# autosome-ru/pasio

Hardware: NVIDIA B200
Metric: whole-contig segmentation throughput, default pasio pipeline (nt/s); DP cell updates/s in dp_cells_per_s (higher is better)
Workload: dtype f64

## Files before the change

include/pasio_b200.h:

```cpp
#ifndef PASIO_B200_H
#define PASIO_B200_H

#include <stdint.h>

#ifdef __cplusplus
extern "C" {
#endif

typedef struct pasio_ctx pasio_ctx;

typedef enum pasio_status {
    PASIO_OK = 0,
    PASIO_E_CUDA = -1,
    PASIO_E_ARG = -2,
    PASIO_E_COUNTS = -3,
    PASIO_E_CANDIDATES = -4,
    PASIO_E_TABLE_TOO_SHORT = -5,
    PASIO_E_STATE = -6,
    PASIO_E_TOO_LARGE = -7,
    PASIO_E_NOMEM = -8
} pasio_status;

enum { PASIO_TAB_LOG = 0,
       PASIO_TAB_LGAMMA = 1,
       PASIO_TAB_LGAMMA_ALPHA = 2   };

enum { PASIO_CONSTRAINT_NONE = 0, PASIO_CONSTRAINT_ZEROS = 1, PASIO_CONSTRAINT_CONSTANTS = 2 };

enum { PASIO_TUNE_WINDOW_PRUNE = 0,
       PASIO_TUNE_WINDOW_PHASES = 1,
       PASIO_TUNE_EXACT_PRUNE = 2,
       PASIO_TUNE_EXACT_LAG = 3,
       PASIO_TUNE_EXACT_RING = 4,
       PASIO_TUNE_LOGFAC_EXACT = 5,
       PASIO_TUNE_WINDOW_SPECULATE = 6,
       PASIO_TUNE_UPLOAD_NARROW = 7,
       PASIO_TUNE_LOGFAC_EAGER = 8,
       PASIO_TUNE_EXACT_NBLOCK = 9,
       PASIO_TUNE_COUNT = 10 };

int pasio_ctx_create(int device, pasio_ctx **out);
int pasio_ctx_destroy(pasio_ctx *ctx);
const char *pasio_last_error(const pasio_ctx *ctx);
int pasio_abi_version(void);

int pasio_set_params(pasio_ctx *ctx, int alpha_is_int, double alpha, double beta,
                     double segment_creation_cost);
int pasio_table_upload(pasio_ctx *ctx, int table_id, const double *values, int64_t n);
int pasio_table_need(const pasio_ctx *ctx, int64_t *n_log, int64_t *n_lgamma, int64_t *n_lgamma_alpha);

int pasio_contig_load(pasio_ctx *ctx, const int64_t *counts, int64_t n,
                      const int64_t *offsets, int64_t n_contigs);
int pasio_contig_load_rle(pasio_ctx *ctx, const int64_t *starts, const int64_t *values,
                          int64_t n_runs, const int64_t *offsets, int64_t n_contigs);
// ... 2 lines not shown

int pasio_contig_load_device(pasio_ctx *ctx, const int64_t *d_counts_device, int64_t n,
                             const int64_t *offsets, int64_t n_contigs);
int pasio_contig_info(const pasio_ctx *ctx, int64_t *n, int64_t *total_count, int64_t *n_contigs);
int pasio_cumsum_at(pasio_ctx *ctx, const int64_t *positions, int64_t m, int64_t *out);

int pasio_candidates_set(pasio_ctx *ctx, const int64_t *cands, int64_t m);
int pasio_candidates_count(const pasio_ctx *ctx, int64_t *m);
int pasio_candidates_download(pasio_ctx *ctx, int64_t *out, int64_t capacity, int64_t *m);

int pasio_filter_candidates(pasio_ctx *ctx, int constraint, int64_t *n_in, int64_t *n_out);

int pasio_round(pasio_ctx *ctx, int64_t window_size, int64_t window_shift, int constraint,
                int64_t *n_in, int64_t *n_out, int64_t *cells);
int pasio_round_stats(const pasio_ctx *ctx, int64_t *cells, int64_t *cells_skipped);
int pasio_exact_task_plan(int64_t n_candidates, int lag, int nblock, int32_t *triples, int64_t cap, int64_t *n_tasks);
int pasio_upload_stats(const pasio_ctx *ctx, int64_t *wire_bytes);
int pasio_set_tuning(pasio_ctx *ctx, int key, int value);
int pasio_rounds(pasio_ctx *ctx, int64_t window_size, int64_t window_shift, int constraint,
                 int64_t max_rounds, int64_t *rounds_done, int64_t *n_out, int64_t *cells,
                 int64_t *sizes, int64_t sizes_cap);
int pasio_set_penalties(pasio_ctx *ctx, const double *split_number_penalty, int64_t n_split_number_penalty,
                        double first_column_refund, const double *length_penalty, int64_t n_length_penalty);

int pasio_square_split(pasio_ctx *ctx, int64_t *out_splits, int64_t cap, int64_t *n_splits,
                       double *score, double *prefix_scores, int64_t *previous_splits);
int pasio_square_split_regularized(pasio_ctx *ctx, const double *length_penalty, int64_t n_length_penalty,
                                   const double *split_number_penalty, int64_t n_split_number_penalty,
                                   double first_column_refund, int64_t *out_splits, int64_t cap, int64_t *n_splits,
                                   double *score, double *prefix_scores, int64_t *previous_splits);
// ... 40 lines not shown
```

pasio_b200/_native.py:

```python
import ctypes
import os
import threading

import numpy as np

_HERE = os.path.dirname(os.path.abspath(__file__))
LIB_PATH = os.environ.get('PASIO_B200_LIB') or os.path.join(_HERE, 'libpasio_b200.so')

OK = 0
E_CUDA, E_ARG, E_COUNTS, E_CANDIDATES, E_TABLE_TOO_SHORT, E_STATE, E_TOO_LARGE, E_NOMEM = range(-1, -9, -1)
TAB_LOG, TAB_LGAMMA, TAB_LGAMMA_ALPHA = 0, 1, 2
CONSTRAINTS = {'none': 0, 'zeros': 1, 'constants': 2}
TUNE = {'window_prune': 0, 'window_phases': 1, 'exact_prune': 2, 'exact_lag': 3, 'exact_ring': 4, 'logfac_exact': 5,
        'window_speculate': 6, 'upload_narrow': 7,
        'logfac_eager': 8, 'exact_nblock': 9}
TIMING_FAMILIES = ['scan', 'window_dp', 'compact', 'exact_dp', 'score', 'h2d', 'd2h']

_i64 = ctypes.c_int64
_i64p = ctypes.POINTER(ctypes.c_int64)
_f64p = ctypes.POINTER(ctypes.c_double)
_vp = ctypes.c_void_p

SIGNATURES = {
    'pasio_ctx_create': (ctypes.c_int, [ctypes.c_int, ctypes.POINTER(_vp)]),
    'pasio_ctx_destroy': (ctypes.c_int, [_vp]),
    'pasio_last_error': (ctypes.c_char_p, [_vp]),
    'pasio_abi_version': (ctypes.c_int, []),
    'pasio_set_params': (ctypes.c_int, [_vp, ctypes.c_int, ctypes.c_double, ctypes.c_double, ctypes.c_double]),
    'pasio_table_upload': (ctypes.c_int, [_vp, ctypes.c_int, _f64p, _i64]),
    'pasio_table_need': (ctypes.c_int, [_vp, _i64p, _i64p, _i64p]),
    'pasio_contig_load': (ctypes.c_int, [_vp, _i64p, _i64, _i64p, _i64]),
    'pasio_contig_load_round': (ctypes.c_int, [_vp, _i64p, _i64, _i64, _i64, ctypes.c_int, _i64p, _i64p, _i64p]),
    'pasio_contig_load_rle': (ctypes.c_int, [_vp, _i64p, _i64p, _i64, _i64p, _i64]),
    'pasio_contig_load_device': (ctypes.c_int, [_vp, _vp, _i64, _i64p, _i64]),
    'pasio_contig_info': (ctypes.c_int, [_vp, _i64p, _i64p, _i64p]),
    'pasio_cumsum_at': (ctypes.c_int, [_vp, _i64p, _i64, _i64p]),
    'pasio_candidates_set': (ctypes.c_int, [_vp, _i64p, _i64]),
    'pasio_candidates_count': (ctypes.c_int, [_vp, _i64p]),
    'pasio_candidates_download': (ctypes.c_int, [_vp, _i64p, _i64, _i64p]),
    'pasio_filter_candidates': (ctypes.c_int, [_vp, ctypes.c_int, _i64p, _i64p]),
    'pasio_round': (ctypes.c_int, [_vp, _i64, _i64, ctypes.c_int, _i64p, _i64p, _i64p]),
    'pasio_round_stats': (ctypes.c_int, [_vp, _i64p, _i64p]),
    'pasio_exact_task_plan': (ctypes.c_int, [_i64, ctypes.c_int, ctypes.c_int, ctypes.POINTER(ctypes.c_int32), _i64, _i64p]),
    'pasio_upload_stats': (ctypes.c_int, [_vp, _i64p]),
    'pasio_set_tuning': (ctypes.c_int, [_vp, ctypes.c_int, ctypes.c_int]),
    'pasio_rounds': (ctypes.c_int, [_vp, _i64, _i64, ctypes.c_int, _i64, _i64p, _i64p, _i64p, _i64p, _i64]),
    'pasio_set_penalties': (ctypes.c_int, [_vp, _f64p, _i64, ctypes.c_double, _f64p, _i64]),
    'pasio_square_split': (ctypes.c_int, [_vp, _i64p, _i64, _i64p, _f64p, _f64p, _i64p]),
    'pasio_square_split_regularized': (ctypes.c_int, [_vp, _f64p, _i64, _f64p, _i64, ctypes.c_double, _i64p, _i64, _i64p, _f64p,
                                                     _f64p, _i64p]),
    'pasio_suffix_scores': (ctypes.c_int, [_vp, _i64, _f64p]),
    'pasio_segment_scores': (ctypes.c_int, [_vp, _f64p, _i64p, _f64p, _f64p, _i64, _i64p]),
    'pasio_segment_scores_sum': (ctypes.c_int, [_vp, _f64p]),
    'pasio_segment_lmm': (ctypes.c_int, [_vp, _f64p, _i64, _f64p]),
    'pasio_logfac_prefetch': (ctypes.c_int, [_vp]),
    'pasio_host_alloc': (ctypes.c_int, [_i64, ctypes.POINTER(_vp)]),
    'pasio_host_free': (ctypes.c_int, [_vp]),
# ... 323 lines not shown
        return n_in.value, n_out.value, cells.value

    def set_tuning(self, key, value):
        self._check(self.lib.pasio_set_tuning(self.ctx, TUNE[key], int(value)))

    def upload_stats(self):
        b = _i64(0)
        self._check(self.lib.pasio_upload_stats(self.ctx, ctypes.byref(b)))
        return b.value

    def round_stats(self):
        a, b = _i64(0), _i64(0)
        self._check(self.lib.pasio_round_stats(self.ctx, ctypes.byref(a), ctypes.byref(b)))
        return a.value, b.value

    def rounds(self, window_size, window_shift, constraint, num_rounds=None, first=None):
        n, _, _ = self.info()
        limit = max(1, n if num_rounds is None else num_rounds)
        self._cands_obj = None
        sizes, cells_total = [], 0
        if first is not None:
            sizes.append(first[0])
            cells_total += first[2]
            limit -= 1
            if first[0] == first[1] or limit == 0:
                return sizes, self.candidate_count(), cells_total
        while limit > 0:
            done, n_out, cells = _i64(0), _i64(0), _i64(0)
            buf = np.zeros(64, dtype=np.int64)
            step = min(limit, 64)
# ... 232 lines not shown
```

pasio_b200/csrc/api.cu:

```cuda
#include "common.cuh"

#include <algorithm>
#include <thread>
#include <atomic>
#include <chrono>
#include <memory>
#include <cstdarg>
#include <cstdlib>
#include <cstdio>
#include <cstring>

static thread_local std::string g_create_error;

int pasio_fail(pasio_ctx *ctx, int code, const char *fmt, ...)
{
    char buf[512];
    va_list ap;
    va_start(ap, fmt);
    vsnprintf(buf, sizeof buf, fmt, ap);
    va_end(ap);
    if (ctx) ctx->err = buf; else g_create_error = buf;
    return code;
}

// ... 372 lines not shown
    if (e != cudaSuccess) return pasio_fail(nullptr, PASIO_E_CUDA, "cudaSetDevice: %s", cudaGetErrorString(e));
    pasio_ctx *ctx = new pasio_ctx();
    ctx->device = device;
    ctx->sm_count = prop.multiProcessorCount;
    ctx->smem_optin = (int)prop.sharedMemPerBlockOptin;
    int prio_lo = 0, prio_hi = 0;
    cudaDeviceGetStreamPriorityRange(&prio_lo, &prio_hi);
    if (cudaStreamCreateWithPriority(&ctx->stream, cudaStreamNonBlocking, prio_hi) != cudaSuccess ||
        cudaStreamCreateWithPriority(&ctx->stream2, cudaStreamNonBlocking, 0) != cudaSuccess ||
        cudaStreamCreateWithFlags(&ctx->stream_copy, cudaStreamNonBlocking) != cudaSuccess ||
        cudaStreamCreateWithPriority(&ctx->stream_lx, cudaStreamNonBlocking, 0) != cudaSuccess ||
        cudaEventCreateWithFlags(&ctx->ev_lx0, cudaEventDisableTiming) != cudaSuccess ||
        cudaEventCreateWithFlags(&ctx->ev_lx1, cudaEventDisableTiming) != cudaSuccess ||
        cudaEventCreateWithFlags(&ctx->ev_fork, cudaEventDisableTiming) != cudaSuccess ||
        cudaEventCreateWithFlags(&ctx->ev_join, cudaEventDisableTiming) != cudaSuccess ||
        cudaMallocHost((void **)&ctx->h_scalars, 16 * sizeof(i64)) != cudaSuccess ||
        pasio_reserve(ctx, ctx->scalars, 16 * sizeof(i64)) != PASIO_OK) {
        g_create_error = "context allocation failed: " + ctx->err;
        delete ctx;
        return PASIO_E_CUDA;
    }
    memset(ctx->h_scalars, 0, 16 * sizeof(i64));
    auto env_int = [](const char *name, int dflt) { const char *v = getenv(name); return v ? atoi(v) : dflt; };
    ctx->tune[PASIO_TUNE_WINDOW_PRUNE] = env_int("PASIO_WD_PRUNE", 1);
    ctx->tune[PASIO_TUNE_WINDOW_PHASES] = env_int("PASIO_WD_PHASES", 1);
    ctx->tune[PASIO_TUNE_EXACT_PRUNE] = env_int("PASIO_XD_PRUNE", 1);
    ctx->tune[PASIO_TUNE_EXACT_LAG] = env_int("PASIO_XD_LAG", 5);
    ctx->tune[PASIO_TUNE_EXACT_RING] = env_int("PASIO_XD_RING", 1);
    ctx->tune[PASIO_TUNE_LOGFAC_EXACT] = env_int("PASIO_B200_EXACT_LMM", 1);
    ctx->tune[PASIO_TUNE_WINDOW_SPECULATE] = env_int("PASIO_WD_SPECULATE", 1);
    ctx->tune[PASIO_TUNE_UPLOAD_NARROW] = env_int("PASIO_B200_UPLOAD_NARROW", 1);
    ctx->tune[PASIO_TUNE_LOGFAC_EAGER] = env_int("PASIO_B200_LOGFAC_EAGER", 0);
    ctx->tune[PASIO_TUNE_EXACT_NBLOCK] = env_int("PASIO_XD_NBLOCK", 3);
    if (ctx->tune[PASIO_TUNE_EXACT_LAG] < 3 || ctx->tune[PASIO_TUNE_EXACT_LAG] > 5) ctx->tune[PASIO_TUNE_EXACT_LAG] = 5;
    *out = ctx;
    return PASIO_OK;
}

extern "C" int pasio_ctx_destroy(pasio_ctx *ctx)
{
    if (!ctx) return PASIO_OK;
    cudaSetDevice(ctx->device);
    cudaStreamSynchronize(ctx->stream);
    drop_borrowed_counts(ctx);
    DevBuf *bufs[] = {&ctx->tab[0], &ctx->tab[1], &ctx->tab[2], &ctx->counts, &ctx->cg, &ctx->cpbits, &ctx->keepbits,
                      &ctx->bounds, &ctx->brank, &ctx->cand[0], &ctx->cand[1], &ctx->candC[0], &ctx->candC[1], &ctx->win_st, &ctx->win_en, &ctx->win_small, &ctx->win_medium, &ctx->win_large, &ctx->win_flags,
                      &ctx->blocksum, &ctx->tilestate, &ctx->scalars, &ctx->dpL, &ctx->dpC, &ctx->dpP, &ctx->dpPrev,
                      &ctx->dpPart, &ctx->dpPartArg, &ctx->dpMark, &ctx->dpJump, &ctx->fscan, &ctx->logfac_full,
// ... 123 lines not shown
    ctx->n_contigs = n_contigs;
    const size_t bit_bytes = (size_t)((n + 1 + 4095) / 4096) * 512 + 16;
    PASIO_TRY(pasio_reserve(ctx, ctx->cg, (size_t)(n + 2) * 8));
    PASIO_TRY(pasio_reserve(ctx, ctx->cpbits, bit_bytes));
    PASIO_TRY(pasio_reserve(ctx, ctx->keepbits, bit_bytes));
    PASIO_TRY(pasio_reserve(ctx, ctx->bounds, (size_t)(n_contigs + 1) * 4));
    PASIO_TRY(pasio_reserve(ctx, ctx->brank, (size_t)(n_contigs + 1) * 4));
    PASIO_TRY(h2d(ctx, ctx->bounds.p, ctx->h_bounds.data(), (size_t)(n_contigs + 1) * 4));
    PASIO_TRY(launch_scan_counts(ctx));
    PASIO_TRY(d2h(ctx, ctx->h_scalars, ctx->scalars.p, 3 * sizeof(i64)));
    if (ctx->h_scalars[1]) return pasio_fail(ctx, PASIO_E_COUNTS, "counts must be >= 0");
    ctx->total = ctx->h_scalars[0];
    ctx->max_count = ctx->h_scalars[2];
    ctx->have_contig = true;
    ctx->implicit_all = true;
    ctx->m = n + 1;
    ctx->cur = 0;
    PASIO_TRY(launch_boundary_ranks(ctx));
    ctx->h_brank = ctx->h_bounds;
    return PASIO_OK;
}

static int check_load_args(pasio_ctx *ctx, int64_t n, const int64_t *offsets, int64_t n_contigs)
{
    if (ctx->logfac_pending) {
        cudaStreamSynchronize(ctx->stream_lx);
        ctx->logfac_pending = false;
    }
    ctx->logfac_ready = false;
    ctx->logfac_eager = false;
// ... 100 lines not shown
    PASIO_TRY(pasio_reserve(ctx, ctx->counts, (size_t)n * 8 + 16));
    ctx->h_bounds.assign({0, (int32_t)n});
    ctx->n_contigs = 1;
    const size_t bit_alloc = (size_t)((n + 1 + 4095) / 4096) * 512 + 16;
    PASIO_TRY(pasio_reserve(ctx, ctx->cg, (size_t)(n + 2) * 8));
    PASIO_TRY(pasio_reserve(ctx, ctx->cpbits, bit_alloc));
    PASIO_TRY(pasio_reserve(ctx, ctx->keepbits, bit_alloc));
    PASIO_TRY(pasio_reserve(ctx, ctx->bounds, 2 * 4));
    PASIO_TRY(pasio_reserve(ctx, ctx->brank, 2 * 4));
    PASIO_TRY(h2d(ctx, ctx->bounds.p, ctx->h_bounds.data(), 2 * 4));
    const size_t bit_bytes = (size_t)((n + 1 + 31) / 32 + 2) * 4;
    CUDA_TRY(ctx, cudaMemsetAsync(ctx->keepbits.p, 0, bit_bytes, ctx->stream));
    i64 n_tiles = 0, tile_elems = 0;
    PASIO_TRY(launch_scan_prepare(ctx, &n_tiles, &tile_elems));
    ctx->implicit_all = true;
    ctx->m = n + 1;
    ctx->cur = 0;
    ctx->n_small = ctx->n_medium = ctx->n_large = -1;

    const i64 chunk_tiles = (i64)(32 << 20) / tile_elems;
    const i64 n_chunks = (n_tiles + chunk_tiles - 1) / chunk_tiles;
    while ((i64)ctx->chunk_events.size() < n_chunks) {
        cudaEvent_t e;
        CUDA_TRY(ctx, cudaEventCreateWithFlags(&e, cudaEventDisableTiming));
        ctx->chunk_events.push_back(e);
    }
    CUDA_TRY(ctx, cudaEventRecord(ctx->ev_fork, ctx->stream));
    CUDA_TRY(ctx, cudaStreamWaitEvent(ctx->stream_copy, ctx->ev_fork, 0));
    i64 queued = 0;
    auto queue_copies = [&](i64 upto) -> int {
// ... 103 lines not shown
        ctx->logfac_pending = true;
        ctx->logfac_eager = true;
    }
    PASIO_TRY(launch_boundary_ranks(ctx));
    ctx->h_brank = ctx->h_bounds;
    if (n_in) *n_in = ctx->m;
    if (n_out) *n_out = ctx->m;
    if (cells) *cells = 0;
    if (table_rc != PASIO_OK) return table_rc;

    const int nxt = 1 - ctx->cur;
    PASIO_TRY(pasio_reserve(ctx, ctx->cand[nxt], (size_t)ctx->m * 4));
    i64 m_new = 0;
    PASIO_TRY(launch_compact_keepbits(ctx, nxt, &m_new));
    PASIO_TRY(d2h(ctx, ctx->h_scalars + 10, ctx->scalars.as<i64>() + 10, 24));
    if (cells) *cells = ctx->h_scalars[10];
    ctx->last_cells = ctx->h_scalars[10];
    ctx->last_cells_skipped = ctx->h_scalars[12];
    ctx->cur = nxt;
    ctx->implicit_all = false;
    ctx->m = m_new;
    if (n_out) *n_out = m_new;
    return refresh_boundary_ranks(ctx);
}

extern "C" int pasio_contig_info(const pasio_ctx *ctx, int64_t *n, int64_t *total_count, int64_t *n_contigs)
{
    if (!ctx || !ctx->have_contig) return PASIO_E_STATE;
    if (n) *n = ctx->n;
    if (total_count) *total_count = ctx->total;
    if (n_contigs) *n_contigs = ctx->n_contigs;
    return PASIO_OK;
}
// ... 29 lines not shown

static int refresh_boundary_ranks(pasio_ctx *ctx)
{
    PASIO_TRY(launch_boundary_ranks(ctx));
    if (ctx->n_contigs > 1) {
        ctx->h_brank.resize((size_t)ctx->n_contigs + 1);
        PASIO_TRY(d2h(ctx, ctx->h_brank.data(), ctx->brank.p, (size_t)(ctx->n_contigs + 1) * 4));
    }
    return PASIO_OK;
}

extern "C" int pasio_candidates_set(pasio_ctx *ctx, const int64_t *cands, int64_t m)
{
    NEED_CTX(ctx);
    if (!ctx->have_contig) return pasio_fail(ctx, PASIO_E_STATE, "no contig loaded");
    if (!cands) {
        ctx->implicit_all = true;
        ctx->m = ctx->n + 1;
        return refresh_boundary_ranks(ctx);
    }
    if (m < 2 || m > ctx->n + 1) return pasio_fail(ctx, PASIO_E_CANDIDATES, "need 2 <= len(candidates) <= n+1");
    PASIO_TRY(pasio_reserve(ctx, ctx->dpJump, (size_t)m * 8));
    PASIO_TRY(pasio_reserve(ctx, ctx->cand[ctx->cur], (size_t)m * 4));
    PASIO_TRY(h2d(ctx, ctx->dpJump.p, cands, (size_t)m * 8));
    i64 *d_bad = ctx->scalars.as<i64>() + 5;
    CUDA_TRY(ctx, cudaMemsetAsync(d_bad, 0, 8, ctx->stream));
    narrow_candidates_kernel<<<ctx->sm_count * 4, 256, 0, ctx->stream>>>(ctx->dpJump.as<i64>(), m, ctx->n,
                                                                        ctx->cand[ctx->cur].as<int32_t>(), d_bad);
    CUDA_TRY(ctx, cudaGetLastError());
    PASIO_TRY(d2h(ctx, ctx->h_scalars + 5, d_bad, 8));
    if (ctx->h_scalars[5]) { ctx->implicit_all = true; ctx->m = ctx->n + 1; return pasio_fail(ctx, PASIO_E_CANDIDATES, "candidate out of range"); }
    ctx->implicit_all = false;
    ctx->m = m;
    PASIO_TRY(pasio_reserve(ctx, ctx->candC[ctx->cur], (size_t)m * 8));
    PASIO_TRY(launch_gather_i64(ctx, ctx->cg.as<i64>(), ctx->cand[ctx->cur].as<int32_t>(), nullptr, m, ctx->candC[ctx->cur].as<i64>()));
    PASIO_TRY(refresh_boundary_ranks(ctx));
    i64 bad = 0;
    PASIO_TRY(launch_validate_candidates(ctx, &bad));
    if (bad) {
        ctx->implicit_all = true;
        ctx->m = ctx->n + 1;
        refresh_boundary_ranks(ctx);
        return pasio_fail(ctx, PASIO_E_CANDIDATES,
                          "candidates must start at 0, end at len(counts), ascend strictly and contain every contig boundary");
    }
    return PASIO_OK;
}

extern "C" int pasio_candidates_count(const pasio_ctx *ctx, int64_t *m)
{
    if (!ctx || !ctx->have_contig || !m) return PASIO_E_STATE;
    *m = ctx->m;
    return PASIO_OK;
}

// ... 12 lines not shown
    if (capacity < ctx->m) return pasio_fail(ctx, PASIO_E_ARG, "capacity %lld < %lld candidates", (long long)capacity, (long long)ctx->m);
    PASIO_TRY(pasio_reserve(ctx, ctx->dpJump, (size_t)ctx->m * 8));
    widen_candidates_kernel<<<ctx->sm_count * 4, 256, 0, ctx->stream>>>(cur_cand(ctx), ctx->m, ctx->dpJump.as<i64>());
    CUDA_TRY(ctx, cudaGetLastError());
    return d2h(ctx, out, ctx->dpJump.p, (size_t)ctx->m * 8);
}

extern "C" int pasio_filter_candidates(pasio_ctx *ctx, int constraint, int64_t *n_in, int64_t *n_out)
{
    NEED_CTX(ctx);
    if (!ctx->have_contig) return pasio_fail(ctx, PASIO_E_STATE, "no contig loaded");
    if (ctx->n_contigs != 1) return pasio_fail(ctx, PASIO_E_STATE, "pasio_filter_candidates works on a single-contig context");
    if (constraint < 0 || constraint > 2) return pasio_fail(ctx, PASIO_E_ARG, "unknown constraint %d", constraint);
    if (n_in) *n_in = ctx->m;
    PASIO_TRY(launch_filter_candidates(ctx, constraint));
    const int nxt = 1 - ctx->cur;
    PASIO_TRY(pasio_reserve(ctx, ctx->cand[nxt], (size_t)ctx->m * 4));
    i64 m_new = 0;
    PASIO_TRY(launch_compact_keepbits(ctx, nxt, &m_new));
    ctx->cur = nxt;
    ctx->implicit_all = false;
    ctx->m = m_new;
    if (n_out) *n_out = m_new;
    return refresh_boundary_ranks(ctx);
}

static int build_window_table(pasio_ctx *ctx, i64 wsize, i64 wshift, i64 *nwin_out)
{
    if (ctx->n_contigs == 1) {
        *nwin_out = (ctx->m - 1 + wshift - 1) / wshift;
// ... 47 lines not shown
                          "contig total %lld / length %lld (m=%lld, implicit=%d, windows=%lld)", (long long)max_cnt,
                          (long long)max_span, (long long)ctx->total, (long long)ctx->n, (long long)ctx->m,
                          (int)ctx->implicit_all, (long long)nwin);
    PASIO_TRY(check_dp_tables(ctx, max_span, max_cnt, true));

    const size_t bit_bytes = (size_t)((ctx->n + 1 + 31) / 32 + 2) * 4;
    CUDA_TRY(ctx, cudaMemsetAsync(ctx->keepbits.p, 0, bit_bytes, ctx->stream));
    if (penalties_on(ctx)) PASIO_TRY(launch_window_dp_reg(ctx, nwin, (int)window_size, (int)window_shift, constraint));
    else PASIO_TRY(launch_window_dp(ctx, nwin, (int)window_size, (int)window_shift, constraint));

    const int nxt = 1 - ctx->cur;
    PASIO_TRY(pasio_reserve(ctx, ctx->cand[nxt], (size_t)ctx->m * 4));
    i64 m_new = 0;
    PASIO_TRY(launch_compact_keepbits(ctx, nxt, &m_new));
    PASIO_TRY(d2h(ctx, ctx->h_scalars + 10, ctx->scalars.as<i64>() + 10, 24));
    if (cells) *cells = ctx->h_scalars[10];
    ctx->last_cells = ctx->h_scalars[10];
    ctx->last_cells_skipped = ctx->h_scalars[12];
    ctx->cur = nxt;
    ctx->implicit_all = false;
    ctx->m = m_new;
    if (n_out) *n_out = m_new;
    return refresh_boundary_ranks(ctx);
}

extern "C" int pasio_rounds(pasio_ctx *ctx, int64_t window_size, int64_t window_shift, int constraint,
                            int64_t max_rounds, int64_t *rounds_done, int64_t *n_out, int64_t *cells,
                            int64_t *sizes, int64_t sizes_cap)
{
    NEED_CTX(ctx);
    if (!ctx->have_contig) return pasio_fail(ctx, PASIO_E_STATE, "no contig loaded");
    i64 limit = max_rounds <= 0 ? ctx->n : max_rounds;
    if (limit < 1) limit = 1;
// ... 17 lines not shown
extern "C" int pasio_upload_stats(const pasio_ctx *ctx, int64_t *wire_bytes)
{
    if (!ctx || !wire_bytes) return PASIO_E_ARG;
    *wire_bytes = ctx->last_wire_bytes;
    return PASIO_OK;
}

extern "C" int pasio_round_stats(const pasio_ctx *ctx, int64_t *cells, int64_t *cells_skipped)
{
    if (!ctx) return PASIO_E_ARG;
    if (cells) *cells = ctx->last_cells;
    if (cells_skipped) *cells_skipped = ctx->last_cells_skipped;
    return PASIO_OK;
}

extern "C" int pasio_set_tuning(pasio_ctx *ctx, int key, int value)
{
    if (!ctx) return PASIO_E_ARG;
    if (key < 0 || key >= PASIO_TUNE_COUNT) return pasio_fail(ctx, PASIO_E_ARG, "unknown tuning key %d", key);
    if (key == PASIO_TUNE_EXACT_LAG && (value < 3 || value > 5)) return pasio_fail(ctx, PASIO_E_ARG, "exact lag must be 3, 4 or 5");
    ctx->tune[key] = value;
    if (key == PASIO_TUNE_LOGFAC_EXACT) {
        if (ctx->logfac_pending) { cudaStreamSynchronize(ctx->stream_lx); ctx->logfac_pending = false; }
        ctx->logfac_ready = false;
        ctx->logfac_eager = false;
    }
    return PASIO_OK;
}

static int finish_square_split(pasio_ctx *ctx, i64 N, int64_t *out_splits, int64_t cap, int64_t *n_splits, double *score,
                               double *prefix_scores, int64_t *previous_splits)
{
    if (score) PASIO_TRY(d2h(ctx, score, ctx->dpP.as<double>() + (N - 1), 8));
    if (prefix_scores) PASIO_TRY(d2h(ctx, prefix_scores, ctx->dpP.p, (size_t)N * 8));
    if (previous_splits) {
        std::vector<int> tmp((size_t)N);
        PASIO_TRY(d2h(ctx, tmp.data(), ctx->dpPrev.p, (size_t)N * 4));
        for (i64 k = 0; k < N; ++k) previous_splits[k] = tmp[(size_t)k];
    }
    PASIO_TRY(launch_backtrace_mark(ctx, N));
    const int nxt = 1 - ctx->cur;
    PASIO_TRY(pasio_reserve(ctx, ctx->cand[nxt], (size_t)N * 4));
    i64 m_new = 0;
    PASIO_TRY(launch_compact_keepbits(ctx, nxt, &m_new));
    ctx->cur = nxt;
    ctx->implicit_all = false;
    ctx->m = m_new;
    PASIO_TRY(refresh_boundary_ranks(ctx));
    if (n_splits) *n_splits = m_new;
    if (out_splits) {
        if (cap < m_new) return pasio_fail(ctx, PASIO_E_ARG, "capacity %lld < %lld splits", (long long)cap, (long long)m_new);
        return pasio_candidates_download(ctx, out_splits, cap, nullptr);
    }
    return PASIO_OK;
}
// ... 314 lines not shown
```

pasio_b200/csrc/common.cuh:

```cuda
#pragma once

#include <cuda_runtime.h>
#include <stdint.h>
#include <string>
#include <vector>

#include "../../include/pasio_b200.h"

typedef long long i64;
typedef unsigned long long u64;

#define PASIO_ABI_VERSION 1

struct DevBuf {
    void *p = nullptr;
    size_t bytes = 0;
    template <typename T> T *as() const { return reinterpret_cast<T *>(p); }
};

enum TimingFamily { TF_SCAN = 0, TF_WINDOW_DP = 1, TF_COMPACT = 2, TF_EXACT_DP = 3, TF_SCORE = 4,
                    TF_H2D = 5, TF_D2H = 6, TF_COUNT = 7 };

struct TimedSpan { int family; cudaEvent_t a, b; };

// ... 62 lines not shown
    DevBuf blocksum, tilestate, scalars, dpL, dpC, dpP, dpPrev, dpPart, dpPartArg, dpMark, dpJump, fscan, logfac_full;
    DevBuf xpRing, xpRec, xpTasks, regLR, regNR;

    bool pen_num = false, pen_len = false;
    DevBuf penNR, penLR;
    i64 n_pen_nr = 0, n_pen_lr = 0;
    double pen_refund = 0.0;
    DevBuf lxPos, lxSum, lxFirst, lxState;
    i64 lx_terms = 0;
    i64 scan_tiles_done = 0;

    int tune[PASIO_TUNE_COUNT];
    i64 *h_scalars = nullptr;

    i64 last_cells = 0, last_cells_skipped = 0;
    std::vector<i64> pw_leaf_start;
    i64 pw_n = -1;
    std::vector<double> pw_leaf_sum;

    bool timing = false;
    std::vector<TimedSpan> spans;
    std::vector<cudaEvent_t> event_pool;
    double fam_ms[TF_COUNT] = {0};
    i64 fam_launches[TF_COUNT] = {0};
};

int pasio_fail(pasio_ctx *ctx, int code, const char *fmt, ...);
int pasio_reserve(pasio_ctx *ctx, DevBuf &b, size_t bytes);

#define CUDA_TRY(ctx, call)                                                                     \
// ... 99 lines not shown
```

pasio_b200/csrc/window_dp.cu:

```cuda
#include "dp_core.cuh"
#include "bound.cuh"
#include <cstdio>
#include <cstdlib>

namespace {

constexpr int WD_THREADS = 256;
constexpr int WD_WARPS = WD_THREADS / 32;
constexpr int WD_FARW = WD_WARPS - 1;
constexpr int NEAR_Q = 4;
constexpr int PR_CB = 32;
constexpr int PR_FB = 8;
constexpr int PR_MIN_N = 256;
constexpr int PR_DENSE = 28;

#ifdef PASIO_WD_PROF
__device__ unsigned long long g_wd_prof[16];
struct ProfAcc { long long t0; long long a0, a1, a2, a3, a4, a5, a6, a7; };
#define PROF_DECL ProfAcc prof = {clock64(), 0, 0, 0, 0, 0, 0, 0, 0}
__device__ __forceinline__ long long prof_clock()
{
    unsigned dummy;
    long long t;
    asm volatile("ld.volatile.shared.u32 %0, [%1];" : "=r"(dummy) : "r"(0u) : "memory");
// ... 30 lines not shown
    int constraint;
    int alpha_int;
    double alpha;
    double pen;
    int cap;
    u64 *cells;
    u64 *cells_skipped;
    unsigned *work_counter;
    const int32_t *list;
    i64 w_begin;
    i64 n_p1, list_len;
    unsigned char *done_flags;
    int p1_stride;
    int skip_covered;
    int speculate;
    int n_lg;
};

__host__ __device__ inline size_t window_smem_bytes(int cap)
{
    const size_t capr = (size_t)((cap + 31) & ~31);
    return capr * 16
           + NEAR_Q * 32 * 8
           + DP_JB * DP_JB * 8
           + NEAR_Q * 32 * 4
           + 24 * 4
           + capr * 2
           + (capr / PR_CB) * sizeof(CoarseRec)
           + 2 * 32 * sizeof(float4)
           + capr * 2
// ... 265 lines not shown
            }
        }
    }
#pragma unroll
    for (int kk = 0; kk < NK; ++kk) {
        const int k = w7 + kk * NW;
        if (k < lane && jb + lane < N) sTri[k * DP_JB + lane] = w[kk];
    }
}

__device__ __forceinline__ void build_coarse_record(int jb, const ColRec *sCol, CoarseRec *rec, double tilt_scale_c,
                                                    double tilt_scale_l)
{
    const ColRec me = sCol[jb + (threadIdx.x & 31)];
    fit_column_record(me.C, me.L, me.P, rec, tilt_scale_c, tilt_scale_l);
}

template <bool AI, int U, int RPL, bool PRUNE>
__global__ void __launch_bounds__(WD_THREADS, 3)
window_dp_kernel(WinDpParams p)
{
    extern __shared__ __align__(16) unsigned char smem[];
    const int capr = (p.cap + 31) & ~31;
    ColRec *sCol = reinterpret_cast<ColRec *>(smem);
    double *sPartV = reinterpret_cast<double *>(sCol + capr);
    double *sTri = sPartV + NEAR_Q * 32;
    int *sPartA = reinterpret_cast<int *>(sTri + DP_JB * DP_JB);
    int *sMisc = sPartA + NEAR_Q * 32;
    unsigned short *sPrev = reinterpret_cast<unsigned short *>(sMisc + 24);
    CoarseRec *sCoarse = reinterpret_cast<CoarseRec *>(sPrev + capr);
// ... 157 lines not shown
            const int par = ((jbn - 1) / DP_JB) & 1;
            const double delta_path = (sScal[0] + sScal[1] + fabs(p.pen) * DP_JB) * 1.8189894035458565e-12;
            compute_row_lb<AI>(jbn - DP_JB, jbn, N, sCol, sRow + 32 * par, sScal + 4 + par, delta_path, p.pen, p.gtab, p.ltab,
                               p.alpha_int, p.alpha);
            if (lane == 0) { sListCount[4 * par] = 0; sListCount[4 * par + 1] = 0; sListCount[4 * par + 2] = 0; }
        };
        auto run_far = [&](int jbf) {
            const int kf = (jbf - 1) / DP_JB, par = kf & 1;
            skipped += far_pass<AI>(jbf, N, kf - 1, sCol, sCoarse, sRow + 32 * par, sScal[4 + par], sList, sList + capr,
                                    sList + capr + capr / PR_CB + 8, sListCount + 4 * par, sFarV + (par * WD_FARW + warp - 1) * 32,
                                    sFarA + (par * WD_FARW + warp - 1) * 32,
                                    far_delta(), p.gtab, p.ltab, p.alpha_int, p.alpha PROF_PASS);
        };
        int jb = 1;
        const bool pipelined = PRUNE && N > PR_MIN_N && p.cand != nullptr;
        for (; jb < N && (!pipelined || jb < 1 + 2 * DP_JB); jb += DP_JB) {
            dp_block_step<AI, WD_WARPS, U, RPL>(jb, N, 0, sCol, sPrev, nullptr, sPartV, sPartA, sTri,
                                                p.gtab, p.ltab, p.alpha_int, p.alpha, p.pen, -INFINITY, 0, 0);
            if (pipelined && warp == 0) finish_block(jb);
        }
        PROF_T(6);
        if (pipelined && jb < N) {
            int spec_wait = 0, spec_back = 1;
            if (warp == 0) prepare_rows(jb);
            __syncthreads();
            if (warp > 0) run_far(jb);
            else if (jb + DP_JB < N) prepare_rows(jb + DP_JB);
            __syncthreads();
            for (; jb < N; jb += DP_JB) {
                const int k = (jb - 1) / DP_JB, buf = k & 1;
// ... 21 lines not shown
                        --spec_wait;
                    }
                    if (!resolved) block_chain<NEAR_Q>(jb, N, sCol, sPrev, nullptr, sPartV, sPartA, sTri, p.pen, ib, ia, 0, nullptr);
                    __syncwarp();
                    finish_block(jb);
                    if (jb + 2 * DP_JB < N) prepare_rows(jb + 2 * DP_JB);
                } else if (jb + DP_JB < N) {
                    run_far(jb + DP_JB);
                }
                PROF_T(2);
                __syncthreads();
                PROF_T(7);
            }
        }

        for (int k = tid; k < N; k += WD_THREADS) sMark[k] = (k == N - 1);
        __syncthreads();
        unsigned short *ja = sPrev, *jb2 = sJump;
        for (int reach = 1; reach < N; reach <<= 1) {
            for (int k = tid; k < N; k += WD_THREADS)
                if (sMark[k]) sMark[ja[k]] = 1;
            for (int k = tid; k < N; k += WD_THREADS) jb2[k] = ja[ja[k]];
            __syncthreads();
            unsigned short *t = ja; ja = jb2; jb2 = t;
        }
        int every = N == nq;
        for (int k = tid; k < N; k += WD_THREADS) {
            if (sMark[k]) {
                const i64 pos = first + sCol[k].L;
                atomicOr(p.keepbits + (pos >> 5), 1u << (pos & 31));
            } else {
                every = 0;
            }
        }
// ... 197 lines not shown
    p.ltab = ctx->tab[PASIO_TAB_LOG].as<double>();
    p.constraint = constraint;
    p.alpha_int = (int)ctx->alpha_int;
    p.alpha = ctx->alpha;
    p.pen = ctx->pen;
    i64 cap = (i64)wsize + 1;
    if (cap > ctx->m) cap = ctx->m;
    if (cap > 8192 || window_smem_bytes((int)cap) > (size_t)ctx->smem_optin)
        return pasio_fail(ctx, PASIO_E_TOO_LARGE, "window of %lld candidates does not fit one CTA's shared memory (max %d)",
                          (long long)cap, window_dp_max_candidates(ctx));
    p.cap = (int)cap;
    p.cells = ctx->scalars.as<u64>() + 10;
    p.cells_skipped = ctx->scalars.as<u64>() + 12;
    p.work_counter = ctx->scalars.as<unsigned>() + 2 * 11;
    p.w_begin = w_begin;
    if (keep_cell_counters) CUDA_TRY(ctx, cudaMemsetAsync(ctx->scalars.as<u64>() + 11, 0, 8, ctx->stream));
    else CUDA_TRY(ctx, cudaMemsetAsync(ctx->scalars.as<u64>() + 10, 0, 24, ctx->stream));
    CUDA_TRY(ctx, cudaMemsetAsync(ctx->scalars.as<u64>() + 15, 0, 8, ctx->stream));

    static const int small_env = getenv("PASIO_WD_SMALL") ? atoi(getenv("PASIO_WD_SMALL")) : 1;
    const int phase_env = ctx->tune[PASIO_TUNE_WINDOW_PHASES];
    const bool use_lists = small_env && ctx->n_small + ctx->n_medium + ctx->n_large == nwin;
    const i64 n_small = use_lists ? ctx->n_small : 0, n_medium = use_lists ? ctx->n_medium : 0;
    const i64 n_large = use_lists ? ctx->n_large : nwin;
    p.list = use_lists ? ctx->win_large.as<int32_t>() : nullptr;
    p.nwin = n_large;
    p.list_len = nwin;
    p.n_p1 = use_lists ? ctx->n_large_p1 : n_large;
    p.skip_covered = phase_env;
    p.speculate = ctx->tune[PASIO_TUNE_WINDOW_SPECULATE];
    p.done_flags = ctx->win_flags.as<unsigned char>();
    p.p1_stride = wshift > 0 && wsize / wshift > 1 ? wsize / wshift : 1;
    if (!use_lists) p.skip_covered = 0;
    ctx->n_small = ctx->n_medium = ctx->n_large = ctx->n_large_p1 = -1;
    TimingScope ts_all(ctx, TF_WINDOW_DP, 0);
    const bool fork = n_small + n_medium > 0 && n_small + n_medium <= 64;
    const bool serial_small = n_small + n_medium > 64;
    if (fork) CUDA_TRY(ctx, cudaEventRecord(ctx->ev_fork, ctx->stream));

    auto launch_small = [&](auto kern, const int32_t *list, i64 n, int nwarps, int ctas, size_t smem_bytes, unsigned *counter,
                            cudaStream_t stream) -> int {
        if (n <= 0) return PASIO_OK;
        WinDpParams ps = p;
        ps.list = list;
        ps.nwin = n;
// ... 84 lines not shown
```

Baseline: 5.706 billion.

## Certify windows where every candidate stays a split, skipping full DP

Adds a certification pass to the pruned window DP. It tries to prove that, in a near-converged round, each candidate's best predecessor is the one right before it. It checks this with coarse and fine bounds plus exact checks on the rows that survive pruning. If the window passes, the full DP and backtrace pointer-jumping are skipped and all candidates are kept. If it fails, the DP resumes from the block where it failed. The pass is enabled by default only when the previous round removed less than 1% of candidates, and it adds per-window overhead plus extra certify-stat counters and a d2h copy.

```diff
diff --git a/include/pasio_b200.h b/include/pasio_b200.h
--- a/include/pasio_b200.h
+++ b/include/pasio_b200.h
@@ -37,7 +37,8 @@
        PASIO_TUNE_UPLOAD_NARROW = 7,
        PASIO_TUNE_LOGFAC_EAGER = 8,
        PASIO_TUNE_EXACT_NBLOCK = 9,
-       PASIO_TUNE_COUNT = 10 };
+       PASIO_TUNE_WINDOW_CERTIFY = 10,
+       PASIO_TUNE_COUNT = 11 };
 
 int pasio_ctx_create(int device, pasio_ctx **out);
 int pasio_ctx_destroy(pasio_ctx *ctx);
@@ -70,6 +71,7 @@
 int pasio_round(pasio_ctx *ctx, int64_t window_size, int64_t window_shift, int constraint,
                 int64_t *n_in, int64_t *n_out, int64_t *cells);
 int pasio_round_stats(const pasio_ctx *ctx, int64_t *cells, int64_t *cells_skipped);
+int pasio_round_certify_stats(const pasio_ctx *ctx, int64_t *passed, int64_t *fell_back, int64_t *resume_rows_sum);
 int pasio_exact_task_plan(int64_t n_candidates, int lag, int nblock, int32_t *triples, int64_t cap, int64_t *n_tasks);
 int pasio_upload_stats(const pasio_ctx *ctx, int64_t *wire_bytes);
 int pasio_set_tuning(pasio_ctx *ctx, int key, int value);
diff --git a/pasio_b200/_native.py b/pasio_b200/_native.py
--- a/pasio_b200/_native.py
+++ b/pasio_b200/_native.py
@@ -13,7 +13,7 @@
 CONSTRAINTS = {'none': 0, 'zeros': 1, 'constants': 2}
 TUNE = {'window_prune': 0, 'window_phases': 1, 'exact_prune': 2, 'exact_lag': 3, 'exact_ring': 4, 'logfac_exact': 5,
         'window_speculate': 6, 'upload_narrow': 7,
-        'logfac_eager': 8, 'exact_nblock': 9}
+        'logfac_eager': 8, 'exact_nblock': 9, 'window_certify': 10}
 TIMING_FAMILIES = ['scan', 'window_dp', 'compact', 'exact_dp', 'score', 'h2d', 'd2h']
 
 _i64 = ctypes.c_int64
@@ -41,6 +41,7 @@
     'pasio_filter_candidates': (ctypes.c_int, [_vp, ctypes.c_int, _i64p, _i64p]),
     'pasio_round': (ctypes.c_int, [_vp, _i64, _i64, ctypes.c_int, _i64p, _i64p, _i64p]),
     'pasio_round_stats': (ctypes.c_int, [_vp, _i64p, _i64p]),
+    'pasio_round_certify_stats': (ctypes.c_int, [_vp, _i64p, _i64p, _i64p]),
     'pasio_exact_task_plan': (ctypes.c_int, [_i64, ctypes.c_int, ctypes.c_int, ctypes.POINTER(ctypes.c_int32), _i64, _i64p]),
     'pasio_upload_stats': (ctypes.c_int, [_vp, _i64p]),
     'pasio_set_tuning': (ctypes.c_int, [_vp, ctypes.c_int, ctypes.c_int]),
@@ -394,6 +395,11 @@
         self._check(self.lib.pasio_round_stats(self.ctx, ctypes.byref(a), ctypes.byref(b)))
         return a.value, b.value
 
+    def round_certify_stats(self):
+        a, b, c = _i64(0), _i64(0), _i64(0)
+        self._check(self.lib.pasio_round_certify_stats(self.ctx, ctypes.byref(a), ctypes.byref(b), ctypes.byref(c)))
+        return a.value, b.value, c.value
+
     def rounds(self, window_size, window_shift, constraint, num_rounds=None, first=None):
         n, _, _ = self.info()
         limit = max(1, n if num_rounds is None else num_rounds)
diff --git a/pasio_b200/csrc/api.cu b/pasio_b200/csrc/api.cu
--- a/pasio_b200/csrc/api.cu
+++ b/pasio_b200/csrc/api.cu
@@ -410,13 +410,13 @@
         cudaEventCreateWithFlags(&ctx->ev_lx1, cudaEventDisableTiming) != cudaSuccess ||
         cudaEventCreateWithFlags(&ctx->ev_fork, cudaEventDisableTiming) != cudaSuccess ||
         cudaEventCreateWithFlags(&ctx->ev_join, cudaEventDisableTiming) != cudaSuccess ||
-        cudaMallocHost((void **)&ctx->h_scalars, 16 * sizeof(i64)) != cudaSuccess ||
-        pasio_reserve(ctx, ctx->scalars, 16 * sizeof(i64)) != PASIO_OK) {
+        cudaMallocHost((void **)&ctx->h_scalars, 20 * sizeof(i64)) != cudaSuccess ||
+        pasio_reserve(ctx, ctx->scalars, 20 * sizeof(i64)) != PASIO_OK) {
         g_create_error = "context allocation failed: " + ctx->err;
         delete ctx;
         return PASIO_E_CUDA;
     }
-    memset(ctx->h_scalars, 0, 16 * sizeof(i64));
+    memset(ctx->h_scalars, 0, 20 * sizeof(i64));
     auto env_int = [](const char *name, int dflt) { const char *v = getenv(name); return v ? atoi(v) : dflt; };
     ctx->tune[PASIO_TUNE_WINDOW_PRUNE] = env_int("PASIO_WD_PRUNE", 1);
     ctx->tune[PASIO_TUNE_WINDOW_PHASES] = env_int("PASIO_WD_PHASES", 1);
@@ -428,6 +428,7 @@
     ctx->tune[PASIO_TUNE_UPLOAD_NARROW] = env_int("PASIO_B200_UPLOAD_NARROW", 1);
     ctx->tune[PASIO_TUNE_LOGFAC_EAGER] = env_int("PASIO_B200_LOGFAC_EAGER", 0);
     ctx->tune[PASIO_TUNE_EXACT_NBLOCK] = env_int("PASIO_XD_NBLOCK", 3);
+    ctx->tune[PASIO_TUNE_WINDOW_CERTIFY] = env_int("PASIO_WD_CERTIFY", 1);
     if (ctx->tune[PASIO_TUNE_EXACT_LAG] < 3 || ctx->tune[PASIO_TUNE_EXACT_LAG] > 5) ctx->tune[PASIO_TUNE_EXACT_LAG] = 5;
     *out = ctx;
     return PASIO_OK;
@@ -581,6 +582,7 @@
     ctx->max_count = ctx->h_scalars[2];
     ctx->have_contig = true;
     ctx->implicit_all = true;
+    ctx->prev_round_in = 0;
     ctx->m = n + 1;
     ctx->cur = 0;
     PASIO_TRY(launch_boundary_ranks(ctx));
@@ -711,6 +713,7 @@
     i64 n_tiles = 0, tile_elems = 0;
     PASIO_TRY(launch_scan_prepare(ctx, &n_tiles, &tile_elems));
     ctx->implicit_all = true;
+    ctx->prev_round_in = 0;
     ctx->m = n + 1;
     ctx->cur = 0;
     ctx->n_small = ctx->n_medium = ctx->n_large = -1;
@@ -844,9 +847,13 @@
     i64 m_new = 0;
     PASIO_TRY(launch_compact_keepbits(ctx, nxt, &m_new));
     PASIO_TRY(d2h(ctx, ctx->h_scalars + 10, ctx->scalars.as<i64>() + 10, 24));
+    PASIO_TRY(d2h(ctx, ctx->h_scalars + 16, ctx->scalars.as<i64>() + 16, 24));
     if (cells) *cells = ctx->h_scalars[10];
     ctx->last_cells = ctx->h_scalars[10];
     ctx->last_cells_skipped = ctx->h_scalars[12];
+    for (int k = 0; k < 3; ++k) ctx->last_certify[k] = ctx->h_scalars[16 + k];
+    ctx->prev_round_in = ctx->m;
+    ctx->prev_round_out = m_new;
     ctx->cur = nxt;
     ctx->implicit_all = false;
     ctx->m = m_new;
@@ -906,8 +913,10 @@
 {
     NEED_CTX(ctx);
     if (!ctx->have_contig) return pasio_fail(ctx, PASIO_E_STATE, "no contig loaded");
+    ctx->prev_round_in = 0;
     if (!cands) {
         ctx->implicit_all = true;
+    ctx->prev_round_in = 0;
         ctx->m = ctx->n + 1;
         return refresh_boundary_ranks(ctx);
     }
@@ -931,6 +940,7 @@
     PASIO_TRY(launch_validate_candidates(ctx, &bad));
     if (bad) {
         ctx->implicit_all = true;
+    ctx->prev_round_in = 0;
         ctx->m = ctx->n + 1;
         refresh_boundary_ranks(ctx);
         return pasio_fail(ctx, PASIO_E_CANDIDATES,
@@ -973,6 +983,7 @@
     if (constraint < 0 || constraint > 2) return pasio_fail(ctx, PASIO_E_ARG, "unknown constraint %d", constraint);
     if (n_in) *n_in = ctx->m;
     PASIO_TRY(launch_filter_candidates(ctx, constraint));
+    ctx->prev_round_in = 0;
     const int nxt = 1 - ctx->cur;
     PASIO_TRY(pasio_reserve(ctx, ctx->cand[nxt], (size_t)ctx->m * 4));
     i64 m_new = 0;
@@ -1050,9 +1061,13 @@
     i64 m_new = 0;
     PASIO_TRY(launch_compact_keepbits(ctx, nxt, &m_new));
     PASIO_TRY(d2h(ctx, ctx->h_scalars + 10, ctx->scalars.as<i64>() + 10, 24));
+    PASIO_TRY(d2h(ctx, ctx->h_scalars + 16, ctx->scalars.as<i64>() + 16, 24));
     if (cells) *cells = ctx->h_scalars[10];
     ctx->last_cells = ctx->h_scalars[10];
     ctx->last_cells_skipped = ctx->h_scalars[12];
+    for (int k = 0; k < 3; ++k) ctx->last_certify[k] = ctx->h_scalars[16 + k];
+    ctx->prev_round_in = ctx->m;
+    ctx->prev_round_out = m_new;
     ctx->cur = nxt;
     ctx->implicit_all = false;
     ctx->m = m_new;
@@ -1100,6 +1115,15 @@
     return PASIO_OK;
 }
 
+extern "C" int pasio_round_certify_stats(const pasio_ctx *ctx, int64_t *passed, int64_t *fell_back, int64_t *resume_rows_sum)
+{
+    if (!ctx) return PASIO_E_ARG;
+    if (passed) *passed = ctx->last_certify[0];
+    if (fell_back) *fell_back = ctx->last_certify[1];
+    if (resume_rows_sum) *resume_rows_sum = ctx->last_certify[2];
+    return PASIO_OK;
+}
+
 extern "C" int pasio_set_tuning(pasio_ctx *ctx, int key, int value)
 {
     if (!ctx) return PASIO_E_ARG;
@@ -1125,6 +1149,7 @@
         for (i64 k = 0; k < N; ++k) previous_splits[k] = tmp[(size_t)k];
     }
     PASIO_TRY(launch_backtrace_mark(ctx, N));
+    ctx->prev_round_in = 0;
     const int nxt = 1 - ctx->cur;
     PASIO_TRY(pasio_reserve(ctx, ctx->cand[nxt], (size_t)N * 4));
     i64 m_new = 0;
diff --git a/pasio_b200/csrc/common.cuh b/pasio_b200/csrc/common.cuh
--- a/pasio_b200/csrc/common.cuh
+++ b/pasio_b200/csrc/common.cuh
@@ -100,6 +100,8 @@
     i64 *h_scalars = nullptr;
 
     i64 last_cells = 0, last_cells_skipped = 0;
+    i64 last_certify[3] = {0, 0, 0};
+    i64 prev_round_in = 0, prev_round_out = 0;
     std::vector<i64> pw_leaf_start;
     i64 pw_n = -1;
     std::vector<double> pw_leaf_sum;
diff --git a/pasio_b200/csrc/window_dp.cu b/pasio_b200/csrc/window_dp.cu
--- a/pasio_b200/csrc/window_dp.cu
+++ b/pasio_b200/csrc/window_dp.cu
@@ -68,6 +68,8 @@
     int p1_stride;
     int skip_covered;
     int speculate;
+    int certify;
+    u64 *certify_stats;
     int n_lg;
 };
 
@@ -363,6 +365,177 @@
 {
     const ColRec me = sCol[jb + (threadIdx.x & 31)];
     fit_column_record(me.C, me.L, me.P, rec, tilt_scale_c, tilt_scale_l);
+}
+
+constexpr int CT_RB = 16;
+
+template <bool AI>
+__device__ __forceinline__ int certify_window(const WinDpParams &p, int N, ColRec *sCol, CoarseRec *sCoarse, const double *sScal0,
+                                              double *sScal1, double *sT, float4 *sRowG, double *sLbAbs, int *sSkip,
+                                              unsigned short *sL1, int *sFail, int *sL1Count, double tilt_c, double tilt_l,
+                                              u64 &skipped)
+{
+    const int tid = threadIdx.x, lane = tid & 31, warp = tid >> 5;
+    const int nrb = (N - 1 + DP_JB - 1) / DP_JB;
+    if (tid == 0) { *sFail = N; *sL1Count = 0; }
+    if (tid < CT_RB) sSkip[tid] = 0;
+    for (int kg = 0; kg < nrb; kg += CT_RB) {
+        const int r0 = 1 + DP_JB * kg, r1 = min(N, r0 + DP_JB * CT_RB), kge = min(nrb, kg + CT_RB);
+        for (int j = r0 + tid; j < r1; j += WD_THREADS) {
+            const int2 me = col_lc(sCol, j), bf = col_lc(sCol, j - 1);
+            sT[j - r0] = self_score<AI>(bf.y, bf.x, make_row<AI>(me.y, me.x, p.alpha_int, p.alpha), p.gtab, p.ltab);
+        }
+        __syncthreads();
+        if (tid == 0) {
+            double P = sCol[r0 - 1].P, mx = *sScal1;
+            for (int j = r0; j < r1; ++j) {
+                const double t = __dadd_rn(sT[j - r0], P);
+                P = __dadd_rn(t, p.pen);
+                sT[j - r0] = t;
+                sCol[j].P = P;
+                mx = fmax(mx, fabs(P));
+            }
+            *sScal1 = mx;
+        }
+        __syncthreads();
+        for (int k = kg + warp; k < kge; k += WD_WARPS) {
+            const int jb = 1 + DP_JB * k;
+            if (jb + DP_JB <= N) build_coarse_record(jb, sCol, sCoarse + k, tilt_c, tilt_l);
+            const bool valid = jb + lane < N;
+            const int j = min(jb + lane, N - 1);
+            const double T = sT[j - r0];
+            const int2 me = col_lc(sCol, j);
+            const RowConst<AI> rme = make_row<AI>(me.y, me.x, p.alpha_int, p.alpha);
+            const int c0 = k == 0 ? 0 : jb - DP_JB;
+            const int dmax = j - c0, dmax_w = __reduce_max_sync(0xffffffffu, dmax);
+            bool ok = fabs(T) < 1e30;
+            constexpr int UN = 4;
+            for (int d = 2; d <= dmax_w; d += UN) {
+                double t[UN];
+#pragma unroll
+                for (int u = 0; u < UN; ++u) {
+                    const ColRec c = sCol[max(j - d - u, 0)];
+                    t[u] = d + u <= dmax ? __dadd_rn(self_score<AI>(c.C, c.L, rme, p.gtab, p.ltab), c.P) : -INFINITY;
+                }
+#pragma unroll
+                for (int u = 0; u < UN; ++u) ok &= t[u] < T;
+            }
+            if (c0 > 0) {
+                const ColRec c = sCol[0];
+                ok &= __dadd_rn(self_score<AI>(c.C, c.L, rme, p.gtab, p.ltab), c.P) < T;
+            }
+            if (valid && !ok) atomicMin(sFail, j);
+            sRowG[(k - kg) * 32 + lane] = make_float4((float)T, (float)me.y, (float)me.x, 0.f);
+            double ab = valid && ok ? fabs(T) : 0.0;
+#pragma unroll
+            for (int off = 16; off > 0; off >>= 1) ab = fmax(ab, __shfl_xor_sync(0xffffffffu, ab, off));
+            if (lane == 0) sLbAbs[k - kg] = ab;
+        }
+        __syncthreads();
+        const double delta = (*sScal0 + *sScal1 + fabs(p.pen) * DP_JB) * 5.684341886080802e-14;
+        {
+            const int f = *sFail;
+            const int kend = min(kge, f >= N ? nrb : (f - 1) / DP_JB), k1 = max(kg, 2);
+            int ntot = 0;
+            for (int k = k1; k < kend; ++k) ntot += k - 1;
+            for (int base = 0; base < ntot; base += WD_THREADS) {
+                const int e = base + tid;
+                bool surv = false;
+                int k = k1, cb = e;
+                if (e < ntot) {
+                    while (cb >= k - 1) { cb -= k - 1; ++k; }
+                    const int jb = 1 + DP_JB * k, nrows = min(DP_JB, N - jb);
+                    const int2 rowF = col_lc(sCol, jb), rowL = col_lc(sCol, jb + nrows - 1);
+                    const CoarseRec *rec = sCoarse + cb;
+                    const int4 ends = *reinterpret_cast<const int4 *>(rec);
+                    const double a1 = rec->a, b1 = rec->b;
+                    const double ub1 = rec->mpt + tilted_box_max<AI>(rowF.y - ends.y, rowL.y - ends.x, rowF.x - ends.w, rowL.x - ends.z,
+                                                                     a1, b1, p.gtab, p.ltab, p.alpha_int, p.alpha);
+                    const double m3 = tilted_row_min(sRowG + (k - kg) * 32, 0, nrows - 1, a1, b1, sLbAbs[k - kg], rowL.y, rowL.x);
+                    surv = !(ub1 - m3 + delta < 0.0);
+                    if (!surv) atomicAdd(sSkip + (k - kg), PR_CB * nrows);
+                }
+                const unsigned mask = __ballot_sync(0xffffffffu, surv);
+                if (mask) {
+                    int slot = 0;
+                    if (lane == 0) slot = atomicAdd(sL1Count, __popc(mask));
+                    slot = __shfl_sync(0xffffffffu, slot, 0);
+                    if (surv) sL1[slot + __popc(mask & ((1u << lane) - 1u))] = (unsigned short)(((k - kg) << 8) | cb);
+                }
+            }
+        }
+        __syncthreads();
+        {
+            const int nl1 = *sL1Count;
+            const int rg = lane >> 2, q = lane & 3, er = lane >> 3, ec = lane & 7;
+            for (int e = warp; e < nl1; e += WD_WARPS) {
+                const int ent = sL1[e], kl = ent >> 8, cb = ent & 255;
+                const int jb = 1 + DP_JB * (kg + kl), nrows = min(DP_JB, N - jb);
+                const int f = __shfl_sync(0xffffffffu, *reinterpret_cast<volatile int *>(sFail), 0);
+                if (f < min(jb + DP_JB, N)) continue;
+                const CoarseRec *rec = sCoarse + cb;
+                const double a = rec->a, b = rec->b;
+                const int rr0 = 4 * rg, rr1 = min(rr0 + 3, nrows - 1);
+                bool surv2 = false;
+                int sk = 0;
+                if (rr0 < nrows) {
+                    const int i0 = 1 + PR_CB * cb + PR_FB * q;
+                    const int2 cF = col_lc(sCol, i0), cL = col_lc(sCol, i0 + PR_FB - 1);
+                    const int2 gF = col_lc(sCol, jb + rr0), gL = col_lc(sCol, jb + rr1);
+                    const double m2 = tilted_box_max<AI>(gF.y - cL.y, gL.y - cF.y, gF.x - cL.x, gL.x - cF.x, a, b,
+                                                         p.gtab, p.ltab, p.alpha_int, p.alpha);
+                    const double m3 = tilted_row_min(sRowG + kl * 32, rr0, rr1, a, b, sLbAbs[kl], gL.y, gL.x);
+                    surv2 = !(rec->mpt8[q] + m2 - m3 + delta < 0.0);
+                    if (!surv2) sk = PR_FB * (rr1 - rr0 + 1);
+                }
+                unsigned m = __ballot_sync(0xffffffffu, surv2);
+                int bad = N;
+                while (m) {
+                    constexpr int UX = 4;
+                    double t[UX], T[UX];
+                    int row[UX];
+#pragma unroll
+                    for (int u = 0; u < UX; ++u) {
+                        t[u] = -INFINITY;
+                        T[u] = 0.0;
+                        row[u] = N;
+                        if (m) {
+                            const int l2 = __ffs(m) - 1;
+                            m &= m - 1;
+                            const int r = 4 * (l2 >> 2) + er;
+                            if (r < nrows) {
+                                row[u] = jb + r;
+                                const int2 rl = col_lc(sCol, jb + r);
+                                const RowConst<AI> rc = make_row<AI>(rl.y, rl.x, p.alpha_int, p.alpha);
+                                const ColRec cc = sCol[1 + PR_CB * cb + PR_FB * (l2 & 3) + ec];
+                                t[u] = __dadd_rn(self_score<AI>(cc.C, cc.L, rc, p.gtab, p.ltab), cc.P);
+                                T[u] = sT[jb + r - r0];
+                            }
+                        }
+                    }
+#pragma unroll
+                    for (int u = 0; u < UX; ++u)
+                        if (row[u] < N && !(t[u] < T[u])) bad = min(bad, row[u]);
+                }
+                if (bad < N) atomicMin(sFail, bad);
+#pragma unroll
+                for (int off = 16; off > 0; off >>= 1) sk += __shfl_xor_sync(0xffffffffu, sk, off);
+                if (lane == 0 && sk) atomicAdd(sSkip + kl, sk);
+            }
+        }
+        __syncthreads();
+        const int f = *sFail;
+        if (tid == 0) {
+            const int kf = f >= N ? nrb : (f - 1) / DP_JB;
+            for (int k = kg; k < kge; ++k) {
+                if (k < kf) skipped += (u64)sSkip[k - kg];
+                sSkip[k - kg] = 0;
+            }
+            *sL1Count = 0;
+        }
+        if (f < N) return f;
+    }
+    return N;
 }
 
 template <bool AI, int U, int RPL, bool PRUNE>
@@ -550,6 +723,28 @@
         };
         int jb = 1;
         const bool pipelined = PRUNE && N > PR_MIN_N && p.cand != nullptr;
+        bool passed = false;
+        if (pipelined && p.certify) {
+            __syncthreads();
+            const int f = certify_window<AI>(p, N, sCol, sCoarse, sScal, sScal + 1, sFarV, reinterpret_cast<float4 *>(sTri), sPartV,
+                                             sPartA, sList, sMisc + 2, sMisc + 3, sScal[2], sScal[3], skipped);
+            passed = f >= N;
+            const int kf = (f - 1) / DP_JB, res = passed || kf < 2 ? 1 : 1 + DP_JB * kf;
+            for (int j = 1 + tid; j < res; j += WD_THREADS) sPrev[j] = (unsigned short)(j - 1);
+            if (warp == 0 && !passed) {
+                double ab = 0.0;
+                for (int j = 1 + lane; j < res; j += 32) ab = fmax(ab, fabs(sCol[j].P));
+#pragma unroll
+                for (int off = 16; off > 0; off >>= 1) ab = fmax(ab, __shfl_xor_sync(0xffffffffu, ab, off));
+                if (lane == 0) sScal[1] = ab;
+            }
+            if (tid == 0) {
+                atomicAdd(p.certify_stats + (passed ? 0 : 1), 1ull);
+                if (res > 1) atomicAdd(p.certify_stats + 2, (u64)(res - 1));
+            }
+            jb = passed ? N : res;
+            __syncthreads();
+        }
         for (; jb < N && (!pipelined || jb < 1 + 2 * DP_JB); jb += DP_JB) {
             dp_block_step<AI, WD_WARPS, U, RPL>(jb, N, 0, sCol, sPrev, nullptr, sPartV, sPartA, sTri,
                                                 p.gtab, p.ltab, p.alpha_int, p.alpha, p.pen, -INFINITY, 0, 0);
@@ -601,10 +796,10 @@
             }
         }
 
-        for (int k = tid; k < N; k += WD_THREADS) sMark[k] = (k == N - 1);
+        for (int k = tid; k < N; k += WD_THREADS) sMark[k] = passed || k == N - 1;
         __syncthreads();
         unsigned short *ja = sPrev, *jb2 = sJump;
-        for (int reach = 1; reach < N; reach <<= 1) {
+        for (int reach = passed ? N : 1; reach < N; reach <<= 1) {
             for (int k = tid; k < N; k += WD_THREADS)
                 if (sMark[k]) sMark[ja[k]] = 1;
             for (int k = tid; k < N; k += WD_THREADS) jb2[k] = ja[ja[k]];
@@ -832,8 +1027,12 @@
     p.cells_skipped = ctx->scalars.as<u64>() + 12;
     p.work_counter = ctx->scalars.as<unsigned>() + 2 * 11;
     p.w_begin = w_begin;
+    p.certify_stats = ctx->scalars.as<u64>() + 16;
     if (keep_cell_counters) CUDA_TRY(ctx, cudaMemsetAsync(ctx->scalars.as<u64>() + 11, 0, 8, ctx->stream));
-    else CUDA_TRY(ctx, cudaMemsetAsync(ctx->scalars.as<u64>() + 10, 0, 24, ctx->stream));
+    else {
+        CUDA_TRY(ctx, cudaMemsetAsync(ctx->scalars.as<u64>() + 10, 0, 24, ctx->stream));
+        CUDA_TRY(ctx, cudaMemsetAsync(p.certify_stats, 0, 24, ctx->stream));
+    }
     CUDA_TRY(ctx, cudaMemsetAsync(ctx->scalars.as<u64>() + 15, 0, 8, ctx->stream));
 
     static const int small_env = getenv("PASIO_WD_SMALL") ? atoi(getenv("PASIO_WD_SMALL")) : 1;
@@ -847,6 +1046,9 @@
     p.n_p1 = use_lists ? ctx->n_large_p1 : n_large;
     p.skip_covered = phase_env;
     p.speculate = ctx->tune[PASIO_TUNE_WINDOW_SPECULATE];
+    const int certify_env = ctx->tune[PASIO_TUNE_WINDOW_CERTIFY];
+    p.certify = certify_env >= 2 ||
+                (certify_env == 1 && ctx->prev_round_in > 0 && (ctx->prev_round_in - ctx->prev_round_out) * 100 < ctx->prev_round_in);
     p.done_flags = ctx->win_flags.as<unsigned char>();
     p.p1_stride = wshift > 0 && wsize / wshift > 1 ? wsize / wshift : 1;
     if (!use_lists) p.skip_covered = 0;
```

Measured after the change: 6.362 billion, median of 6. 11.5% higher.
